# fabiocarrara/neural-ode-features

Measured on AMD Instinct MI355X. Metric: images/sec (fwd+adjoint) CIFAR-10 ODE-ResNet bs=128 at 1/2/4/8 GPU, higher is better.
Workload: dtype f32

## Files before the change

neural-ode-features_amd/csrc/kernels_pointwise.hip:

```cpp
#include "node_internal.h"
#include "wino4.h"
#include "step_control.h"
#include <cstring>
#include "../../include/node_hip.h"

namespace node {


__device__ inline float wave_sum(float v) {
#pragma unroll
  for (int off = 32; off > 0; off >>= 1) v += __shfl_xor(v, off, 64);
  return v;
}
__device__ inline float wave_max(float v) {
#pragma unroll
  for (int off = 32; off > 0; off >>= 1) v = fmaxf(v, __shfl_xor(v, off, 64));
  return v;
}

__device__ inline float block_sum_256(float v, float* red ) {
  v = wave_sum(v);
  __syncthreads();
  if ((threadIdx.x & 63) == 0) red[threadIdx.x >> 6] = v;
  __syncthreads();
// ... 298 lines not shown
struct ErrSegs { ErrSeg seg[3]; float* partial[3]; };
__device__ void error_norm_body(const ErrSeg& seg, const Ctrl* ctrl, float rtol, float atol, float* partial);
__global__ __launch_bounds__(256) void k_error_norm(ErrSegs a, const Ctrl* ctrl, float rtol, float atol) {
  if (ctrl->done) return;
  error_norm_body(a.seg[blockIdx.y], ctrl, rtol, atol, a.partial[blockIdx.y]);
}
__device__ void error_norm_body(const ErrSeg& seg, const Ctrl* ctrl, float rtol, float atol, float* partial) {
  __shared__ float red[4];
  const float dtf = (float)ctrl->dt;
  float ce[7], cb[7];
#pragma unroll
  for (int j = 0; j < 7; ++j) { ce[j] = dtf * c_CERR[j]; cb[j] = dtf * c_CSOL[j]; }
  float acc = 0.f;
  const size_t n4 = seg.n >> 2;
  const size_t stride = (size_t)gridDim.x * 256;
  for (size_t v = (size_t)blockIdx.x * 256 + threadIdx.x; v < n4; v += stride) {
    const size_t off = v * 4;
    float4 kv[7];
#pragma unroll
    for (int j = 0; j < 7; ++j) kv[j] = (j == 1) ? make_float4(0, 0, 0, 0) : ld4(seg.k[j] + off);
    const float4 y0 = ld4(seg.y0 + off);
    float4 y1;
    if (seg.compute_y1) {
      float4 s;
      s.x = cb[0] * kv[0].x; s.y = cb[0] * kv[0].y; s.z = cb[0] * kv[0].z; s.w = cb[0] * kv[0].w;
#pragma unroll
      for (int j = 2; j < 6; ++j) { s.x += cb[j] * kv[j].x; s.y += cb[j] * kv[j].y; s.z += cb[j] * kv[j].z; s.w += cb[j] * kv[j].w; }
      y1 = make_float4(y0.x + s.x, y0.y + s.y, y0.z + s.z, y0.w + s.w);
      st4(seg.y1 + off, y1);
    } else {
// ... 384 lines not shown
  if (!fin) {
    for (int sg = 0; sg < a.nseg; ++sg) {
      const size_t n4 = a.n[sg] >> 2;
      float4* y = reinterpret_cast<float4*>(a.y[sg]);
      const float4* y1 = reinterpret_cast<const float4*>(a.y1[sg]);
      float4* k0 = reinterpret_cast<float4*>(a.k0[sg]);
      const float4* k6 = reinterpret_cast<const float4*>(a.k6[sg]);
      for (size_t i = start; i < n4; i += stride) { y[i] = y1[i]; k0[i] = k6[i]; }
      for (size_t i = (n4 << 2) + start; i < a.n[sg]; i += stride) { a.y[sg][i] = a.y1[sg][i]; a.k0[sg][i] = a.k6[sg][i]; }
    }
    return;
  }
  const float dt = (float)c->dt_used;
  const float t0f = (float)c->t_prev, t1f = (float)c->t;
  const float x = ((float)a.targets[0] - t0f) / (t1f - t0f);
  for (int sg = 0; sg < a.nseg; ++sg)
    for (size_t i = start; i < a.n[sg]; i += stride) {
      float kk[7];
#pragma unroll
      for (int q = 0; q < 7; ++q) kk[q] = (q == 1) ? 0.f : a.k[sg][q][i];
      a.y[sg][i] = interp_one(a.y[sg][i], a.y1[sg][i], kk, dt, x);
    }
}
void launch_commit(const CommitArgs& a, hipStream_t s) {
  size_t nmax = 0;
  for (int i = 0; i < a.nseg; ++i) nmax = a.n[i] > nmax ? a.n[i] : nmax;
  size_t blocks = (nmax / 4 + 255) / 256;
  if (blocks > 2048) blocks = 2048;
  if (blocks < 1) blocks = 1;
  hipLaunchKernelGGL(k_commit, dim3((unsigned)blocks), dim3(256), 0, s, a);
}

__global__ void k_set_target(double* targets, double t_end) { targets[0] = t_end; }
void launch_set_target(double* targets, double t_end, hipStream_t s) {
  hipLaunchKernelGGL(k_set_target, dim3(1), dim3(1), 0, s, targets, t_end);
}
__global__ void k_export_record(const Ctrl* c, node_step_record* r, float* miss_flag, int expect) {
// ... 206 lines not shown
  if (cl == 0) {
    __hip_atomic_store(counter, 0u, __ATOMIC_RELAXED, __HIP_MEMORY_SCOPE_AGENT);
    if (a.write_scalar) a.ctrl->ts_k[a.kidx] = a.osign * tot;
    if (a.vjp_t_out) *a.vjp_t_out = a.osign * tot;
  }
}

void launch_theta_finalize(const Dims& d, const ThetaFinalizeArgs& a, hipStream_t s) {
  size_t wblocks = (9 * (size_t)d.C * d.C / 4 + 255) / 256;
  if (a.dU != nullptr) wblocks = ((size_t)d.C * d.C / 4 + 255) / 256;
  if (wblocks > 1024) wblocks = 1024;
  const size_t nsmall = (9 * (size_t)d.C + 63) / 64;
  hipLaunchKernelGGL(k_theta_finalize, dim3((unsigned)(5 * nsmall + 2 * wblocks)), dim3(256), 0, s, a, d);
}

__global__ __launch_bounds__(256) void k_lincomb(Comb c, const Ctrl* ctrl, float* out, size_t n) {
  const float scale = comb_scale(c, ctrl);
  float cf[7];
#pragma unroll
  for (int j = 0; j < 7; ++j) cf[j] = scale * c.coef[j];
  const size_t stride = (size_t)gridDim.x * 256;
  for (size_t i = (size_t)blockIdx.x * 256 + threadIdx.x; i < n; i += stride) {
    float s = 0.f;
    for (int j = 0; j < c.nk; ++j) s += cf[j] * c.k[j][i];
    out[i] = c.y[i] + s;
  }
}
void launch_lincomb(const Comb& c, const Ctrl* ctrl, float* out, size_t n, hipStream_t s) {
  size_t blocks = (n + 255) / 256;
  if (blocks > 2048) blocks = 2048;
// ... 5 lines not shown
```

neural-ode-features_amd/csrc/node_api.hip:

```cpp
#include "node_internal.h"
#include "wino4.h"
#include "../../include/node_hip.h"

#include <cmath>
#include <cstdarg>
#include <cstdio>
#include <cstring>
#include <cstdlib>
#include <atomic>
#include <mutex>
#include <utility>
#include <vector>

using namespace node;

static thread_local char g_err[512] = "";
static int fail(int code, const char* fmt, ...) {
  va_list ap;
  va_start(ap, fmt);
  vsnprintf(g_err, sizeof(g_err), fmt, ap);
  va_end(ap);
  return code;
}
namespace node {
// ... 202 lines not shown
  unsigned* tcount;
  void* thand;
  float *W4V, *W4M;
  float* w4u[4];
  unsigned short* w4ub[4];
  float* tmapS[2];
  W4Scales* w4sc;
  float* W4Va0b;
  float *W4Va[2], *W4Z[2], *W4dU;
  float *act1b, *xh1b, *r1b;
  float *A, *A1, *KA[7];
  float *TH, *TH1, *KT[7];
  float *xh1, *xh2, *xh3, *r1, *r2, *r3;
  float *dz1, *dz2, *G;
  float *wpart[2], *spart[2], *gpart[3], *sred, *wtime[2];
  float* dots;
  double* targets;
  double* forced;
  double* dtlog;
  size_t bytes;
};
constexpr int STEP_LIST_CAP = 4096;

struct Bump {
  char* base;
  size_t off;
  explicit Bump(void* b) : base((char*)b), off(0) {}
  template <typename T>
  T* take(size_t count) {
    off = (off + 255) & ~(size_t)255;
    T* p = (T*)(base + off);
    off += count * sizeof(T);
    return p;
  }
};

Plan make_plan(const Dims& d, int adjoint, int n_t, void* base) {
  Plan p;
  memset(&p, 0, sizeof(p));
  Bump b(base);
  p.ctrl = b.take<Ctrl>(1);
  p.arrive = b.take<unsigned>(4);
  p.targets = b.take<double>((size_t)(n_t > 0 ? n_t : 1));
  p.forced = b.take<double>(STEP_LIST_CAP);
  p.dtlog = b.take<double>(STEP_LIST_CAP);
  for (int i = 0; i < 3; ++i) p.partial[i] = b.take<float>(ERR_BLOCKS * 2);
  const size_t wsz = conv_packed_elems(d);
  for (int i = 0; i < 2; ++i) p.wf[i] = b.take<float>(wsz);
  for (int i = 0; i < 2; ++i) p.tmap[i] = b.take<float>((size_t)d.HW * d.C);
  p.Y = b.take<float>(d.numel);
// ... 46 lines not shown
    p.r3 = b.take<float>((size_t)d.N * d.G);
    p.dz1 = b.take<float>(d.numel + d.C);
    p.dz2 = b.take<float>(d.numel + d.C);
    p.G = b.take<float>(d.numel);
    for (int i = 0; i < 2; ++i) {
      p.wpart[i] = b.take<float>((size_t)d.nsplit * 9 * d.C * d.C);
      p.spart[i] = b.take<float>(prow * 9 * d.C);
    }
    p.sred = b.take<float>((size_t)2 * 9 * d.C + 2 * ((9 * (size_t)d.C + 63) / 64) + 4);
    for (int i = 0; i < 2; ++i) p.wtime[i] = b.take<float>((size_t)9 * d.C);
    const size_t grows = prow > (size_t)d.mtiles ? prow : (size_t)d.mtiles;
    p.gpart[0] = b.take<float>(grows * 2 * d.C);
    p.gpart[1] = b.take<float>(grows * 2 * d.C);
    p.gpart[2] = b.take<float>(prow * 2 * d.C);
    p.dots = b.take<float>((size_t)(n_t > 0 ? n_t : 1));
  }
  p.bytes = ((b.off + 255) & ~(size_t)255);
  return p;
}

struct HostStage {
  Ctrl* ctrl = nullptr;
  double* lists = nullptr;
  size_t cap = 0;
};
thread_local HostStage g_stage;

int get_stage(size_t doubles, HostStage** out) {
  if (!g_stage.ctrl) HIP_TRY(hipHostMalloc((void**)&g_stage.ctrl, sizeof(Ctrl), hipHostMallocDefault));
  if (g_stage.cap < doubles) {
// ... 92 lines not shown
    if (resident) {
      hipStreamCaptureStatus cs = hipStreamCaptureStatusNone;
      if (hipStreamIsCapturing(st, &cs) != hipSuccess) { (void)hipGetLastError(); cs = hipStreamCaptureStatusNone; }
      if (cs != hipStreamCaptureStatusNone) resident = false;
    }
    if (resident && g_resident_cooldown.load(std::memory_order_relaxed) > 0) {
      g_resident_cooldown.fetch_sub(1, std::memory_order_relaxed);
      resident = false;
    }
  }
  bool w4_b16 = false;
  bool w4_f16 = false;
  bool w4_f16_aug = false;
  SideStream* side = nullptr;
  bool side_pending = false;
  float* va0_of(int set) const { return (set && p.W4Va0b != nullptr) ? p.W4Va0b : p.W4Va[0]; }
  bool g_ready = false;
  bool f16_now() const { return w4_f16 && (!aug || g_ready); }
  bool v_ready = false;
  int cur = 0;
  float* act1_of(int i) const { return i ? p.act1b : p.act1; }
  float* xh1_of(int i) const { return i ? p.xh1b : p.xh1; }
  float* r1_of(int i) const { return i ? p.r1b : p.r1; }
  void to_state(const float* nchw, float* dst) {
    if (w4) launch_w4s_from_nchw(nchw, dst, d.N, d.C, d.w4q, st);
    else launch_nchw_to_nhwc(d, nchw, dst, st);
  }
  void from_state(const float* src, float* nchw) {
    if (w4) launch_w4s_to_nchw(src, nchw, d.N, d.C, d.w4q, st);
    else launch_nhwc_to_nchw(d, src, nchw, st);
// ... 60 lines not shown
    if (tiny_mode() && !w4) {
      launch_tiny_pack(d, prm.conv1_w, p.wtiny[0], st);
      launch_tiny_pack(d, prm.conv2_w, p.wtiny[1], st);
      launch_fill(reinterpret_cast<float*>(p.tcount), 0.f, (size_t)d.N * d.G, st);
    }
    if (w4) {
      w4_b16 = w4_uses_bf16(d.N8, d.C);
      w4_f16 = w4_b16 && w4_f16_fits(d.N8, d.C) && (!aug || (w4_f16_aug && w4_wgrad_on() && w4_wgrad_f16_fits(d.N8, d.C)));
      g_ready = false;
      side = nullptr; side_pending = false;
      if (w4_f16 && aug) {
        const char* e = getenv("NODE_TUNE_W4_WGRAD_SIDE");
        if ((e ? atoi(e) : 0) != 0 && !get_side(&side)) side = nullptr;
      }
      if (w4_f16) { zr[nz] = reinterpret_cast<float*>(p.w4sc); zn[nz++] = sizeof(W4Scales) / sizeof(float); }
    }
    launch_time_prep(d, prm.conv1_w, prm.conv2_w, p.tmap[0], p.tmap[1], aug ? p.wtime[0] : nullptr, aug ? p.wtime[1] : nullptr, zr, zn,
                     nz, st);
    if (w4) {
      W4PackJobs jobs;
      memset(&jobs, 0, sizeof(jobs));
      const float* ws_[4] = {prm.conv1_w, prm.conv2_w, prm.conv1_w, prm.conv2_w};
      if (w4_f16) {
        W4ScaleJobs sj;
        memset(&sj, 0, sizeof(sj));
        sj.w[0] = prm.conv1_w; sj.w[1] = prm.conv2_w; sj.wn = (size_t)d.C * (d.C + 1) * 9;
        sj.gb[0] = prm.norm1_w; sj.gb[1] = prm.norm1_b; sj.gb[2] = prm.norm2_w; sj.gb[3] = prm.norm2_b;
        sj.C = d.C; sj.gn_m = d.cpg * d.HW; sj.sc = p.w4sc;
        launch_w4_scales(sj, st);
      }
// ... 107 lines not shown
    launch_w4s_pass(head, tail, a, st);
  }
  int eval_w4(const Comb& cy, float* y_out, const EvalTime& et, float* kY_out, bool train, const Comb* ca, float* a_out,
              float* kA_out, float* kT_out, int kidx, float csign, float* vjp_t_out, bool need_theta, const NextComb* next) {
    const bool do_aug = ca != nullptr;
    if (next != nullptr)
      for (int j = 0; j + 1 < next->cy.nk; ++j)
        if (next->cy.k[j] == kY_out || (do_aug && next->cy.k[j] == kA_out)) next = nullptr;
    if (!v_ready) {
      W4sArgs a = w4_args();
      w4_tail_combine(a, cy, y_out, train, cur, 0);
      w4_pass(0, 1, a);
    }
    v_ready = false;
    const bool wg4 = do_aug && w4_wgrad_on();
    w4_gemm(0, wg4 ? va0_of(cur) : nullptr);
    {
      W4sArgs a = w4_args();
      a.h.M = p.W4M; a.h.bias = prm.conv1_b; a.h.tmapS = p.tmapS[0]; a.h.et = et; a.h.gamma = prm.norm2_w; a.h.beta = prm.norm2_b;
      a.h.osign = 1.f; a.h.relu = 1;
      if (train) { a.h.out_nhwc = wg4 ? nullptr : p.act2; a.h.xhat_s = p.xh2; a.h.rstd = p.r2; }
      a.V = wg4 ? p.W4Va[1] : p.W4V;
      if (f16_now()) a.v_exp = &p.w4sc->e[W4_E_V2];
      w4_pass(1, 0, a);
    }
    w4_gemm(1, wg4 ? p.W4Va[1] : nullptr);
    W4sArgs a3 = w4_args();
    a3.h.M = p.W4M; a3.h.bias = prm.conv2_b; a3.h.tmapS = p.tmapS[1]; a3.h.et = et; a3.h.gamma = prm.norm3_w; a3.h.beta = prm.norm3_b;
    a3.h.osign = et.tsign; a3.h.relu = 0; a3.h.out_s = kY_out;
    if (!do_aug) {
      if (next != nullptr) {
        const int self = next->cy.nk > 0 && next->cy.k[next->cy.nk - 1] == kY_out;
        w4_tail_combine(a3, next->cy, next->y_out, false, cur, self);
        w4_pass(1, 1, a3);
        v_ready = true;
      } else {
        w4_pass(1, 0, a3);
      }
      if (count_nfe) nfe += 1;
      return check_launch("odefunc forward (F(4x4,3x3))");
    }
    a3.t.comb = *ca; a3.t.csign = csign; a3.t.y_out = a_out; a3.t.gpart = p.gpart[2]; a3.t.spart = p.spart[1];
    if (wg4) a3.t.z_out = need_theta ? p.W4Z[1] : nullptr;
    else a3.t.act_nhwc = p.dz2;
    a3.V = p.W4V;
    if (w4_f16) a3.gstat = p.w4sc;
    if (f16_now()) { a3.v_exp = &p.w4sc->e[W4_E_G]; a3.z_exp = &p.w4sc->e[W4_E_G]; }
    w4_pass(1, 2, a3);
    if (count_nfe) nfe += 1;
    w4_gemm(3);
    {
      W4sArgs a = w4_args();
      a.h.M = p.W4M; a.h.gamma = prm.norm2_w; a.h.beta = prm.norm2_b; a.h.xhat_s = p.xh2; a.h.rstd = p.r2; a.h.osign = 1.f;
      a.h.gpart = p.gpart[1]; a.h.spart = p.spart[0];
      if (wg4) a.h.z_out = need_theta ? p.W4Z[0] : nullptr;
      else a.h.out_nhwc = p.dz1;
      a.V = p.W4V;
      if (w4_f16) a.gstat = p.w4sc;
      if (f16_now()) { a.v_exp = &p.w4sc->e[W4_E_G]; a.z_exp = &p.w4sc->e[W4_E_G]; }
      w4_pass(2, 0, a);
    }
    if (need_theta && wg4 && f16_now()) {
      hipStream_t ws = st;
      if (side != nullptr) {
        (void)hipEventRecord(side->fork, st);
        (void)hipStreamWaitEvent(side->s, side->fork, 0);
        ws = side->s;
      }
      {
        ProfScope ps(1, 2.0 * conv_flops(), ws);
        launch_w4_wgrad_f16(reinterpret_cast<const unsigned*>(va0_of(cur)), reinterpret_cast<const unsigned*>(p.W4Z[0]), reinterpret_cast<const unsigned*>(p.W4Va[1]),
                            reinterpret_cast<const unsigned*>(p.W4Z[1]), p.W4dU, p.ctrl, d.N8, d.C, &p.w4sc->e[W4_E_V1], &p.w4sc->e[W4_E_V2], &p.w4sc->e[W4_E_G], ws);
      }
      if (side != nullptr) { (void)hipEventRecord(side->join, side->s); side_pending = true; }
    } else if (need_theta && wg4) {
      W4WgradArgs wa;
      memset(&wa, 0, sizeof(wa));
      wa.V1 = va0_of(cur); wa.Z1 = p.W4Z[0]; wa.V2 = p.W4Va[1]; wa.Z2 = p.W4Z[1]; wa.dU = p.W4dU; wa.ctrl = p.ctrl; wa.N = d.N8; wa.C = d.C;
      ProfScope ps(1, 2.0 * conv_flops(), st);
      launch_w4_wgrad(wa, st);
    } else if (need_theta) {
      WgradArgs w1;
      memset(&w1, 0, sizeof(w1));
      w1.act = act1_of(cur); w1.dz = p.dz1; w1.wpart = p.wpart[0]; w1.ctrl = p.ctrl;
      if (d.wgrad_pair) { w1.act2 = p.act2; w1.dz2 = p.dz2; w1.wpart2 = p.wpart[1]; }
      { ProfScope ps(1, (d.wgrad_pair ? 2.0 : 1.0) * conv_flops(), st); launch_wgrad(d, w1, st); }
      if (!d.wgrad_pair) {
        WgradArgs w2 = w1;
        w2.act = p.act2; w2.dz = p.dz2; w2.wpart = p.wpart[1];
        { ProfScope ps(1, conv_flops(), st); launch_wgrad(d, w2, st); }
      }
    }
    w4_gemm(2);
    {
      W4sArgs a = w4_args();
      a.h.M = p.W4M; a.h.gamma = prm.norm1_w; a.h.beta = prm.norm1_b; a.h.xhat_s = xh1_of(cur); a.h.rstd = r1_of(cur);
      a.h.osign = et.tsign; a.h.out_s = kA_out; a.h.gpart = p.gpart[0];
      if (next != nullptr) {
        w4_tail_combine(a, next->cy, next->y_out, true, cur ^ 1, 0);
        w4_pass(2, 1, a);
        cur ^= 1;
        v_ready = true;
      } else {
        w4_pass(2, 0, a);
      }
    }
    if (!need_theta) return check_launch("augmented dynamics (F(4x4,3x3))");
    if (side_pending) { (void)hipStreamWaitEvent(st, side->join, 0); side_pending = false; }
    ThetaFinalizeArgs tf;
    memset(&tf, 0, sizeof(tf));
    tf.dU = wg4 ? p.W4dU : nullptr;
    tf.wpart[0] = p.wpart[0]; tf.wpart[1] = p.wpart[1];
    tf.spart[0] = p.spart[0]; tf.spart[1] = p.spart[1];
    tf.gpart[0] = p.gpart[0]; tf.gpart[1] = p.gpart[1]; tf.gpart[2] = p.gpart[2];
    tf.gpart_rows[0] = tf.gpart_rows[1] = tf.gpart_rows[2] = tf.spart_rows = d.N * d.w4q;
    tf.wtime[0] = p.wtime[0]; tf.wtime[1] = p.wtime[1]; tf.sred = p.sred;
    tf.et = et; tf.osign = et.tsign; tf.theta_out = kT_out;
    tf.ctrl = p.ctrl; tf.kidx = kidx; tf.write_scalar = kidx >= 0 ? 1 : 0; tf.vjp_t_out = vjp_t_out;
    launch_theta_finalize(d, tf, st);
    return check_launch("augmented dynamics (F(4x4,3x3))");
  }

  int eval_fwd(const Comb& cy, float* y_out, const EvalTime& et, float* k_out, bool train, const NextComb* next = nullptr) {
// ... 171 lines not shown
    return check_launch("initial step");
  }

  struct StepIO {
    int n_targets = 0;
    int n_forced = 0;
    int log_cap = 0;
    float* y_out = nullptr;
  };

  int enqueue_step(const StepIO& io) {
    static int skip_k2 = -1;
    if (skip_k2 < 0) { const char* e = getenv("NODE_TUNE_SKIP_K2_THETA"); skip_k2 = e ? atoi(e) : 1; }
    const bool was_counting = count_nfe;
    count_nfe = false;
    for (int s = 0; s < 6; ++s) {
      const int rc = eval_sys(s + 1, DP_BETA[s], s + 1, SC_DT, et_stage(DP_ALPHA[s]), s == 5, !(skip_k2 && s == 0),
                              s < 5 ? DP_BETA[s + 1] : nullptr, s + 2, s + 1 == 5);
      if (rc != NODE_OK) { count_nfe = was_counting; return rc; }
    }
    count_nfe = was_counting;
    const int nseg = aug ? 3 : 1;
    ErrSeg es[3];
    es[0].y0 = p.Y; es[0].y1 = p.Y1; es[0].n = d.numel; es[0].compute_y1 = 0;
    for (int j = 0; j < 7; ++j) es[0].k[j] = p.KY[j];
    if (aug) {
      es[1] = es[0];
      es[1].y0 = p.A; es[1].y1 = p.A1;
      for (int j = 0; j < 7; ++j) es[1].k[j] = p.KA[j];
      es[2].y0 = p.TH; es[2].y1 = p.TH1; es[2].n = d.P; es[2].compute_y1 = 1;
      for (int j = 0; j < 7; ++j) es[2].k[j] = p.KT[j];
    }
    StepCtlArgs sc;
    memset(&sc, 0, sizeof(sc));
    sc.ctrl = p.ctrl;
    sc.partial[0] = p.partial[0]; sc.partial[1] = p.partial[1]; sc.partial[2] = p.partial[2];
    sc.numel[0] = (double)d.numel; sc.numel[1] = (double)d.numel; sc.numel[2] = (double)d.P;
    sc.nseg = nseg; sc.has_scalar = aug ? 1 : 0; sc.rtol = rtol; sc.atol = atol;
    sc.targets = p.targets; sc.n_targets = io.n_targets;
    sc.forced = io.n_forced > 0 ? p.forced : nullptr; sc.n_forced = io.n_forced;
    sc.dt_log = io.log_cap > 0 ? p.dtlog : nullptr; sc.dt_log_cap = io.log_cap;
    sc.interp_scalar = aug ? 1 : 0;
    sc.w4sc = (aug && w4_f16) ? p.w4sc : nullptr;
    if (nr_fn == nullptr && fold_ctl()) {
      launch_error_norm_ctl(es, p.partial, nseg, sc, p.arrive, st);
    } else {
// ... 6 lines not shown
      ea.ctrl = p.ctrl; ea.targets = p.targets; ea.y0 = p.Y; ea.y1 = p.Y1;
      for (int j = 0; j < 7; ++j) ea.k[j] = p.KY[j];
      ea.y_out = io.y_out;
      if (w4) launch_w4s_emit_outputs(d, ea, st);
      else launch_emit_outputs(d, ea, st);
    }
    CommitArgs cm;
    memset(&cm, 0, sizeof(cm));
    cm.ctrl = p.ctrl; cm.targets = p.targets; cm.nseg = nseg; cm.interp_final = aug ? 1 : 0;
    cm.y[0] = p.Y; cm.y1[0] = p.Y1; cm.k0[0] = p.KY[0]; cm.k6[0] = p.KY[6]; cm.n[0] = d.numel;
    for (int j = 0; j < 7; ++j) cm.k[0][j] = p.KY[j];
    if (aug) {
      cm.y[1] = p.A; cm.y1[1] = p.A1; cm.k0[1] = p.KA[0]; cm.k6[1] = p.KA[6]; cm.n[1] = d.numel;
      cm.y[2] = p.TH; cm.y1[2] = p.TH1; cm.k0[2] = p.KT[0]; cm.k6[2] = p.KT[6]; cm.n[2] = d.P;
      for (int j = 0; j < 7; ++j) { cm.k[1][j] = p.KA[j]; cm.k[2][j] = p.KT[j]; }
    }
    launch_commit(cm, st);
    return check_launch("dopri5 step");
  }

  int run_steps(const StepIO& io, long long max_steps, int guess, int* status) {
    long long enq = 0;
    long long batch = guess > 0 ? guess : 1;
    for (;;) {
      if (batch > max_steps - enq) batch = max_steps - enq;
      for (long long i = 0; i < batch; ++i) TRY(enqueue_step(io));
      enq += batch;
      TRY(readback());
      if (hctrl->status != 0) { *status = hctrl->status; return NODE_OK; }
      if (hctrl->done) return NODE_OK;
// ... 840 lines not shown
  hipStream_t st = (hipStream_t)stream;
  const int nseg = f->nseg, aug = f->has_scalar ? 1 : 0;
  if (method == NODE_METHOD_RK4) {
    const double cf[4] = {1.0 / 8, 3.0 / 8, 3.0 / 8, 1.0 / 8};
    for (int i = 0; i < nseg; ++i) {
      float* ks[7];
      for (int j = 0; j < 7; ++j) ks[j] = f->seg[i].k[j];
      launch_lincomb(Solver::make_comb(f->seg[i].y, ks, cf, 4, SC_DT), p.ctrl, f->seg[i].y1, f->seg[i].n, st);
      HIP_TRY(hipMemcpyAsync(f->seg[i].y, f->seg[i].y1, f->seg[i].n * sizeof(float), hipMemcpyDeviceToDevice, st));
    }
    if (aug) launch_set_scalar_state(p.ctrl, 0.f, 1, st);
    return flat_launch_ok("node_flat_finish_step(rk4)");
  }
  if (method != NODE_METHOD_DOPRI5) return fail(NODE_ERR_ARG, "unknown method %d", method);
  ErrSeg es[3];
  for (int i = 0; i < nseg; ++i) {
    es[i].y0 = f->seg[i].y; es[i].y1 = f->seg[i].y1; es[i].n = f->seg[i].n; es[i].compute_y1 = 0;
    for (int j = 0; j < 7; ++j) es[i].k[j] = f->seg[i].k[j];
  }
  launch_error_norm(es, p.partial, nseg, p.ctrl, f->rtol, f->atol, st);
  StepCtlArgs sc;
  memset(&sc, 0, sizeof(sc));
  sc.ctrl = p.ctrl;
  for (int i = 0; i < nseg; ++i) { sc.partial[i] = p.partial[i]; sc.numel[i] = (double)f->seg[i].n; }
  sc.nseg = nseg; sc.has_scalar = aug; sc.rtol = f->rtol; sc.atol = f->atol;
  sc.targets = p.targets; sc.n_targets = f->n_targets; sc.interp_scalar = aug;
  launch_step_controller(sc, st);
  if (y_out != nullptr) {
    EmitArgs ea;
    ea.ctrl = p.ctrl; ea.targets = p.targets; ea.y0 = f->seg[0].y; ea.y1 = f->seg[0].y1;
// ... 139 lines not shown
```

neural-ode-features_amd/csrc/node_internal.h:

```cpp
#pragma once
#include <hip/hip_runtime.h>
#include <stdint.h>
#include <stddef.h>

namespace node {

constexpr int KCH = 32;
constexpr int BN = 64;
constexpr int WG_THREADS = 256;

struct Dims {
  int N, C, H, W, HW, G, cpg;
  float eps;
  int Wp, Hp, SLOTS;
  int MARGIN;
  int BNE;
  int ntile;
  int nchunk;
  int BM;
  int S;
  int wino;
  int wgrad_wino;
  int wut;
  int tiny;
// ... 75 lines not shown
};
__device__ inline float comb_scale(const Comb& c, const Ctrl* ctrl) {
  return c.scale_mode == SC_ABS ? 1.0f : (c.scale_mode == SC_DT ? (float)ctrl->dt : ctrl->h0);
}

__device__ constexpr float DP_CMID_F[7] = {
    (float)(6025192743.0 / 30085553152.0 / 2.0), 0.f, (float)(51252292925.0 / 65400821598.0 / 2.0),
    (float)(-2691868925.0 / 45128329728.0 / 2.0), (float)(187940372067.0 / 1594534317056.0 / 2.0),
    (float)(-1776094331.0 / 19743644256.0 / 2.0), (float)(11237099.0 / 235043384.0 / 2.0)};
__device__ inline float interp_one(float y0, float y1, const float* k, float dt, float x) {
  float s = (dt * DP_CMID_F[0]) * k[0];
#pragma unroll
  for (int j = 2; j < 7; ++j) s += (dt * DP_CMID_F[j]) * k[j];
  const float ymid = y0 + s;
  const float f0 = k[0], f1 = k[6];
  const float ca = (-2.f * dt) * f0 + (2.f * dt) * f1 + -8.f * y0 + -8.f * y1 + 16.f * ymid;
  const float cb = (5.f * dt) * f0 + (-3.f * dt) * f1 + 18.f * y0 + 14.f * y1 + -32.f * ymid;
  const float cc = (-4.f * dt) * f0 + dt * f1 + -11.f * y0 + -5.f * y1 + 16.f * ymid;
  const float cd = dt * f0;
  const float x2 = x * x, x3 = x2 * x, x4 = x3 * x;
  return ca * x4 + cb * x3 + cc * x2 + cd * x + y0;
}

constexpr int MAX_DEVICES = 64;
inline void allow_full_lds(const void* fn, bool (&done)[MAX_DEVICES]) {
  int dev = 0;
  (void)hipGetDevice(&dev);
  const bool tracked = dev >= 0 && dev < MAX_DEVICES;
  if (tracked && done[dev]) return;
  if (hipFuncSetAttribute(fn, hipFuncAttributeMaxDynamicSharedMemorySize, 160 * 1024) != hipSuccess)
// ... 81 lines not shown
  const float* gamma;
  float* dz_out;
  float* gpart;
  float* spart;
  const float* mask_act;
  float osign;
};
void launch_gn_bwd(const Dims& d, const GnBwdArgs& a, hipStream_t s);

struct ErrSeg {
  const float* y0;
  float* y1;
  const float* k[7];
  size_t n;
  int compute_y1;
};
constexpr int ERR_BLOCKS = 512;
void launch_error_norm(const ErrSeg* segs, float* const* partial , int nseg, const Ctrl* ctrl, float rtol, float atol, hipStream_t s);
struct StepCtlArgs;
void launch_error_norm_ctl(const ErrSeg* segs, float* const* partial, int nseg, const StepCtlArgs& ctl, unsigned* arrive, hipStream_t s);

struct StepCtlArgs {
  Ctrl* ctrl;
  const float* partial[3];
  double numel[3];
  int nseg;
  int has_scalar;
  float rtol, atol;
  const double* targets;
  int n_targets;
// ... 24 lines not shown
  const float* y0; const float* y1; const float* k[7];
  float* y_out;
};
void launch_emit_outputs(const Dims& d, const EmitArgs& a, hipStream_t s);
void launch_emit_flat(const EmitArgs& a, size_t n, hipStream_t s);
void launch_flat_time(const EvalTime& et, float* out, hipStream_t s);
void launch_flat_scalar(Ctrl* ctrl, int which, const float* src, float scale, int accumulate, hipStream_t s);
struct CommitArgs {
  const Ctrl* ctrl;
  const double* targets;
  int nseg;
  float* y[3]; const float* y1[3]; float* k0[3]; const float* k6[3];
  const float* k[3][7];
  size_t n[3];
  int interp_final;
};
void launch_commit(const CommitArgs& a, hipStream_t s);
void launch_set_interval(Ctrl* ctrl, double t, double dt, hipStream_t s);
void launch_set_target(double* targets, double t_end, hipStream_t s);
}
struct node_step_record;
namespace node {
void launch_export_record(const Ctrl* ctrl, node_step_record* rec, float* miss_flag, int expect_steps, hipStream_t s);

struct InitSeg { const float* y0; const float* f0; const float* f1; size_t n; };
void launch_init_norms(const InitSeg* segs, float* const* partial , int nseg, float rtol, float atol, int phase, hipStream_t s);
struct InitCtlArgs;
void launch_init_norms_ctl(const InitSeg* segs, float* const* partial, int nseg, const InitCtlArgs& ctl, unsigned* arrive, hipStream_t s);
struct InitCtlArgs {
  Ctrl* ctrl;
// ... 73 lines not shown
  const float* spart[2];
  const float* gpart[3];
  int gpart_rows[3];
  int spart_rows;
  const float* wtime[2];
  float* sred;
  EvalTime et;
  float osign;
  float* theta_out;
  Ctrl* ctrl;
  int kidx;
  int write_scalar;
  float* vjp_t_out;
};
void launch_theta_finalize(const Dims& d, const ThetaFinalizeArgs& a, hipStream_t s);

struct TinyConvArgs {
  const float* act;
  const unsigned short* wq;
  const float* bias; const float* tmap;
  EvalTime et;
  const float* gamma; const float* beta;
  float* out;
  float* part; unsigned* counter;
  const Ctrl* ctrl;
  int relu; float osign;
  int nx_on, nx_self;
  Comb nx; float* nx_y_out; const float* nx_gamma; const float* nx_beta; float* nx_act;
};
struct TinyResidentArgs {
// ... 54 lines not shown
```

Before: 28120.

## Batch theta finalize across Dopri5 stages into one fused step kernel

In the adjoint step, the per-stage theta-gradient finalize (Winograd dU back-transform plus GN and bias reductions) is deferred. Each stage writes into its own slot buffers, and one kernel then reduces all five stages at once and emits theta1, the error, the midpoint combination and k6 directly. The error-norm and commit kernels gain fast paths that read these precomputed err and mid arrays instead of reloading all seven k vectors for theta. This removes five per-stage finalize launches and repeated passes over the parameter-sized buffers, at the cost of extra workspace per stage and a gfx950-only fence-free hand-off.

```diff
diff --git a/neural-ode-features_amd/csrc/kernels_pointwise.hip b/neural-ode-features_amd/csrc/kernels_pointwise.hip
--- a/neural-ode-features_amd/csrc/kernels_pointwise.hip
+++ b/neural-ode-features_amd/csrc/kernels_pointwise.hip
@@ -336,6 +336,28 @@
   float acc = 0.f;
   const size_t n4 = seg.n >> 2;
   const size_t stride = (size_t)gridDim.x * 256;
+  if (seg.err != nullptr) {
+    for (size_t v = (size_t)blockIdx.x * 256 + threadIdx.x; v < n4; v += stride) {
+      const size_t off = v * 4;
+      const float4 y0 = ld4(seg.y0 + off), y1 = ld4(seg.y1 + off), e = ld4(seg.err + off);
+      float r;
+      r = e.x / (atol + rtol * fmaxf(fabsf(y0.x), fabsf(y1.x))); acc += r * r;
+      r = e.y / (atol + rtol * fmaxf(fabsf(y0.y), fabsf(y1.y))); acc += r * r;
+      r = e.z / (atol + rtol * fmaxf(fabsf(y0.z), fabsf(y1.z))); acc += r * r;
+      r = e.w / (atol + rtol * fmaxf(fabsf(y0.w), fabsf(y1.w))); acc += r * r;
+      acc += 0.f * (((y0.x + y0.y) + (y0.z + y0.w)) + ((y1.x + y1.y) + (y1.z + y1.w)));
+    }
+    if (blockIdx.x == 0)
+      for (size_t i = (n4 << 2) + threadIdx.x; i < seg.n; i += 256) {
+        const float y0 = seg.y0[i], y1 = seg.y1[i];
+        const float r = seg.err[i] / (atol + rtol * fmaxf(fabsf(y0), fabsf(y1)));
+        acc += r * r;
+        acc += 0.f * (y0 + y1);
+      }
+    const float tot = block_sum_256(acc, red);
+    if (threadIdx.x == 0) __hip_atomic_store(&partial[blockIdx.x], tot, __ATOMIC_RELAXED, __HIP_MEMORY_SCOPE_AGENT);
+    return;
+  }
   for (size_t v = (size_t)blockIdx.x * 256 + threadIdx.x; v < n4; v += stride) {
     const size_t off = v * 4;
     float4 kv[7];
@@ -750,13 +772,19 @@
   const float dt = (float)c->dt_used;
   const float t0f = (float)c->t_prev, t1f = (float)c->t;
   const float x = ((float)a.targets[0] - t0f) / (t1f - t0f);
-  for (int sg = 0; sg < a.nseg; ++sg)
+  for (int sg = 0; sg < a.nseg; ++sg) {
+    if (a.mid[sg] != nullptr) {
+      for (size_t i = start; i < a.n[sg]; i += stride)
+        a.y[sg][i] = interp_mid(a.y[sg][i], a.y1[sg][i], a.k[sg][0][i], a.k[sg][6][i], a.mid[sg][i], dt, x);
+      continue;
+    }
     for (size_t i = start; i < a.n[sg]; i += stride) {
       float kk[7];
 #pragma unroll
       for (int q = 0; q < 7; ++q) kk[q] = (q == 1) ? 0.f : a.k[sg][q][i];
       a.y[sg][i] = interp_one(a.y[sg][i], a.y1[sg][i], kk, dt, x);
     }
+  }
 }
 void launch_commit(const CommitArgs& a, hipStream_t s) {
   size_t nmax = 0;
@@ -993,6 +1021,174 @@
   hipLaunchKernelGGL(k_theta_finalize, dim3((unsigned)(5 * nsmall + 2 * wblocks)), dim3(256), 0, s, a, d);
 }
 
+__device__ const float c_W4_GF[6][3] = {{(float)W4_G[0][0], (float)W4_G[0][1], (float)W4_G[0][2]}, {(float)W4_G[1][0], (float)W4_G[1][1], (float)W4_G[1][2]},
+                                        {(float)W4_G[2][0], (float)W4_G[2][1], (float)W4_G[2][2]}, {(float)W4_G[3][0], (float)W4_G[3][1], (float)W4_G[3][2]},
+                                        {(float)W4_G[4][0], (float)W4_G[4][1], (float)W4_G[4][2]}, {(float)W4_G[5][0], (float)W4_G[5][1], (float)W4_G[5][2]}};
+__device__ inline void theta_step_emit(const ThetaStepArgs& a, size_t idx, const float* k, float dtf) {
+  const float k0 = a.k0[idx];
+  float sb = c_CSOL[0] * k0, se = c_CERR[0] * k0, sm = DP_CMID_F[0] * k0;
+#pragma unroll
+  for (int s = 0; s < TH_STAGES; ++s) { sb += c_CSOL[2 + s] * k[s]; se += c_CERR[2 + s] * k[s]; sm += DP_CMID_F[2 + s] * k[s]; }
+  a.th1[idx] = a.th[idx] + dtf * sb;
+  a.err[idx] = dtf * se;
+  a.mid[idx] = dtf * sm;
+  a.k6[idx] = k[TH_STAGES - 1];
+}
+__global__ __launch_bounds__(256) void k_theta_finalize_step(ThetaStepArgs a, Dims d) {
+  if (a.ctrl->done) return;
+  __shared__ float red[TH_STAGES][256];
+  __shared__ int s_last;
+  const ThetaLayout L = theta_layout(d.C);
+  const int C = d.C;
+  const float dtf = (float)a.ctrl->dt;
+  const int nsm = (9 * C + 63) / 64;
+  const int bx_all = blockIdx.x;
+  const int wb = ((int)gridDim.x - 5 * nsm) / 2;
+  if (bx_all >= 5 * nsm) {
+    const int layer = (bx_all - 5 * nsm) / wb, bx = (bx_all - 5 * nsm) - layer * wb;
+    const size_t CC = (size_t)C * C, cc2 = CC / 2;
+    const size_t stride = (size_t)wb * 256;
+    const size_t base = L.wc[layer];
+    for (size_t i = (size_t)bx * 256 + threadIdx.x; i < cc2; i += stride) {
+      float2 ob[9], oe[9], om[9], o6[9];
+#pragma unroll
+      for (int q = 0; q < 9; ++q) ob[q] = oe[q] = om[q] = o6[q] = make_float2(0.f, 0.f);
+#pragma unroll 1
+      for (int xi = 0; xi < 6; ++xi) {
+        float2 ub[6], ue[6], um[6], u6[6];
+#pragma unroll
+        for (int nu = 0; nu < 6; ++nu) ub[nu] = ue[nu] = um[nu] = u6[nu] = make_float2(0.f, 0.f);
+#pragma unroll
+        for (int s = 0; s < TH_STAGES; ++s)
+#pragma unroll
+          for (int nu = 0; nu < 6; ++nu) {
+            const float2 u = reinterpret_cast<const float2*>(a.dU[s] + (size_t)layer * W4_COMPS * CC)[(size_t)(xi * 6 + nu) * cc2 + i];
+            ub[nu].x += c_CSOL[2 + s] * u.x; ub[nu].y += c_CSOL[2 + s] * u.y;
+            ue[nu].x += c_CERR[2 + s] * u.x; ue[nu].y += c_CERR[2 + s] * u.y;
+            um[nu].x += DP_CMID_F[2 + s] * u.x; um[nu].y += DP_CMID_F[2 + s] * u.y;
+            if (s == TH_STAGES - 1) u6[nu] = u;
+          }
+        const float gh[3] = {c_W4_GF[xi][0], c_W4_GF[xi][1], c_W4_GF[xi][2]};
+#pragma unroll
+        for (int kw = 0; kw < 3; ++kw) {
+          float2 tb = make_float2(0.f, 0.f), te = tb, tm = tb, t6 = tb;
+#pragma unroll
+          for (int nu = 0; nu < 6; ++nu) {
+            const float gq = (float)W4_G[nu][kw];
+            if (gq != 0.f) {
+              tb.x += gq * ub[nu].x; tb.y += gq * ub[nu].y; te.x += gq * ue[nu].x; te.y += gq * ue[nu].y;
+              tm.x += gq * um[nu].x; tm.y += gq * um[nu].y; t6.x += gq * u6[nu].x; t6.y += gq * u6[nu].y;
+            }
+          }
+#pragma unroll
+          for (int kh = 0; kh < 3; ++kh) {
+            const int q = kh * 3 + kw;
+            ob[q].x += gh[kh] * tb.x; ob[q].y += gh[kh] * tb.y; oe[q].x += gh[kh] * te.x; oe[q].y += gh[kh] * te.y;
+            om[q].x += gh[kh] * tm.x; om[q].y += gh[kh] * tm.y; o6[q].x += gh[kh] * t6.x; o6[q].y += gh[kh] * t6.y;
+          }
+        }
+      }
+#pragma unroll
+      for (int q = 0; q < 9; ++q) {
+        const size_t idx = base + (size_t)q * CC + 2 * i;
+        const float2 k0 = *reinterpret_cast<const float2*>(a.k0 + idx), th = *reinterpret_cast<const float2*>(a.th + idx);
+        float2 v;
+        v.x = th.x + dtf * (c_CSOL[0] * k0.x + a.tsign * ob[q].x); v.y = th.y + dtf * (c_CSOL[0] * k0.y + a.tsign * ob[q].y);
+        *reinterpret_cast<float2*>(a.th1 + idx) = v;
+        v.x = dtf * (c_CERR[0] * k0.x + a.tsign * oe[q].x); v.y = dtf * (c_CERR[0] * k0.y + a.tsign * oe[q].y);
+        *reinterpret_cast<float2*>(a.err + idx) = v;
+        v.x = dtf * (DP_CMID_F[0] * k0.x + a.tsign * om[q].x); v.y = dtf * (DP_CMID_F[0] * k0.y + a.tsign * om[q].y);
+        *reinterpret_cast<float2*>(a.mid + idx) = v;
+        v.x = a.tsign * o6[q].x; v.y = a.tsign * o6[q].y;
+        *reinterpret_cast<float2*>(a.k6 + idx) = v;
+      }
+    }
+    return;
+  }
+  const int job = bx_all / nsm, bxs = bx_all - job * nsm;
+  const bool gn = job < 3;
+  const int layer = gn ? job : job - 3;
+  const int ncol = gn ? 2 * C : 9 * C;
+  if (bxs * 64 >= ncol) return;
+  const int rows = a.rows;
+  const int cl = threadIdx.x & 63, rg = threadIdx.x >> 6;
+  const int col = bxs * 64 + cl;
+#pragma unroll
+  for (int s = 0; s < TH_STAGES; ++s) {
+    const float* src = gn ? a.gpart[s][layer] : a.spart[s][layer];
+    float v = 0.f;
+    if (col < ncol) {
+      int r = rg;
+      for (; r + 12 < rows; r += 16) {
+        const float v0 = src[(size_t)r * ncol + col], v1 = src[(size_t)(r + 4) * ncol + col];
+        const float v2 = src[(size_t)(r + 8) * ncol + col], v3 = src[(size_t)(r + 12) * ncol + col];
+        v += (v0 + v1) + (v2 + v3);
+      }
+      for (; r < rows; r += 4) v += src[(size_t)r * ncol + col];
+    }
+    red[s][threadIdx.x] = v;
+  }
+  __syncthreads();
+  if (rg != 0) return;
+  const bool on = col < ncol;
+  float v[TH_STAGES], k[TH_STAGES];
+#pragma unroll
+  for (int s = 0; s < TH_STAGES; ++s) v[s] = (red[s][cl] + red[s][64 + cl]) + (red[s][128 + cl] + red[s][192 + cl]);
+  if (gn) {
+    if (on) {
+      const int which = col >= C ? 1 : 0;
+#pragma unroll
+      for (int s = 0; s < TH_STAGES; ++s) k[s] = a.tsign * v[s];
+      theta_step_emit(a, (which ? L.b[layer] : L.g[layer]) + (col - which * C), k, dtf);
+    }
+    return;
+  }
+  if (on) {
+    const float tf = (float)a.ctrl->t;
+#pragma unroll
+    for (int s = 0; s < TH_STAGES; ++s) k[s] = a.tsign * (v[s] * (a.tsign * (tf + a.alpha[s] * dtf)));
+    theta_step_emit(a, L.wt[layer] + col, k, dtf);
+    if (col >= 4 * C && col < 5 * C) {
+#pragma unroll
+      for (int s = 0; s < TH_STAGES; ++s) k[s] = a.tsign * v[s];
+      theta_step_emit(a, L.cb[layer] + (col - 4 * C), k, dtf);
+    }
+  }
+  const int nb = nsm;
+  float* dotpart = a.dotpart;
+  unsigned* counter = reinterpret_cast<unsigned*>(dotpart + TH_STAGES * 2 * nb);
+  const float wt = on ? a.wtime[layer][col] : 0.f;
+  float part[TH_STAGES];
+#pragma unroll
+  for (int s = 0; s < TH_STAGES; ++s) part[s] = wave_sum(on ? v[s] * wt : 0.f);
+#if defined(__HIP_DEVICE_COMPILE__) && !defined(__gfx950__)
+#error "k_theta_finalize_step's fence-free hand-off is only valid on gfx950: use release/acquire on the counter elsewhere"
+#endif
+  if (cl == 0) {
+#pragma unroll
+    for (int s = 0; s < TH_STAGES; ++s)
+      __hip_atomic_store(dotpart + (s * 2 + layer) * nb + bxs, part[s], __ATOMIC_RELAXED, __HIP_MEMORY_SCOPE_AGENT);
+    asm volatile("s_waitcnt vmcnt(0)" ::: "memory");
+    s_last = __hip_atomic_fetch_add(counter, 1u, __ATOMIC_RELAXED, __HIP_MEMORY_SCOPE_AGENT) == (unsigned)(2 * nb - 1);
+  }
+  __builtin_amdgcn_wave_barrier();
+  if (!s_last) return;
+  for (int s = 0; s < TH_STAGES; ++s) {
+    float tot = 0.f;
+    for (int i = cl; i < 2 * nb; i += 64) tot += __hip_atomic_load(dotpart + s * 2 * nb + i, __ATOMIC_RELAXED, __HIP_MEMORY_SCOPE_AGENT);
+    tot = wave_sum(tot);
+    if (cl == 0) a.ctrl->ts_k[2 + s] = a.tsign * tot;
+  }
+  if (cl == 0) __hip_atomic_store(counter, 0u, __ATOMIC_RELAXED, __HIP_MEMORY_SCOPE_AGENT);
+}
+
+void launch_theta_finalize_step(const Dims& d, const ThetaStepArgs& a, hipStream_t s) {
+  size_t wblocks = ((size_t)d.C * d.C / 2 + 255) / 256;
+  if (wblocks > 1024) wblocks = 1024;
+  const size_t nsmall = (9 * (size_t)d.C + 63) / 64;
+  hipLaunchKernelGGL(k_theta_finalize_step, dim3((unsigned)(5 * nsmall + 2 * wblocks)), dim3(256), 0, s, a, d);
+}
+
 __global__ __launch_bounds__(256) void k_lincomb(Comb c, const Ctrl* ctrl, float* out, size_t n) {
   const float scale = comb_scale(c, ctrl);
   float cf[7];
diff --git a/neural-ode-features_amd/csrc/node_api.hip b/neural-ode-features_amd/csrc/node_api.hip
--- a/neural-ode-features_amd/csrc/node_api.hip
+++ b/neural-ode-features_amd/csrc/node_api.hip
@@ -240,6 +240,7 @@
   float *xh1, *xh2, *xh3, *r1, *r2, *r3;
   float *dz1, *dz2, *G;
   float *wpart[2], *spart[2], *gpart[3], *sred, *wtime[2];
+  float *dUs[TH_STAGES], *sparts[TH_STAGES][2], *gparts[TH_STAGES][3], *THerr, *THmid, *thdot;
   float* dots;
   double* targets;
   double* forced;
@@ -260,6 +261,8 @@
     return p;
   }
 };
+
+static bool theta_batch_fits(const Dims& d) { return d.wino4 && d.C % 128 == 0 && d.C < 512; }
 
 Plan make_plan(const Dims& d, int adjoint, int n_t, void* base) {
   Plan p;
@@ -336,6 +339,18 @@
     p.gpart[1] = b.take<float>(grows * 2 * d.C);
     p.gpart[2] = b.take<float>(prow * 2 * d.C);
     p.dots = b.take<float>((size_t)(n_t > 0 ? n_t : 1));
+    if (theta_batch_fits(d) && p.W4dU != nullptr) {
+      for (int s = 0; s < TH_STAGES; ++s) {
+        p.dUs[s] = b.take<float>(w4_du_elems(d.C));
+        for (int i = 0; i < 2; ++i) p.sparts[s][i] = b.take<float>(prow * 9 * d.C);
+        p.gparts[s][0] = b.take<float>(grows * 2 * d.C);
+        p.gparts[s][1] = b.take<float>(grows * 2 * d.C);
+        p.gparts[s][2] = b.take<float>(prow * 2 * d.C);
+      }
+      p.THerr = b.take<float>(d.P);
+      p.THmid = b.take<float>(d.P);
+      p.thdot = b.take<float>((size_t)TH_STAGES * 2 * ((9 * (size_t)d.C + 63) / 64) + 4);
+    }
   }
   p.bytes = ((b.off + 255) & ~(size_t)255);
   return p;
@@ -458,6 +473,8 @@
   bool w4_f16_aug = false;
   SideStream* side = nullptr;
   bool side_pending = false;
+  bool theta_batch = false;
+  int th_slot = -1;
   float* va0_of(int set) const { return (set && p.W4Va0b != nullptr) ? p.W4Va0b : p.W4Va[0]; }
   bool g_ready = false;
   bool f16_now() const { return w4_f16 && (!aug || g_ready); }
@@ -548,6 +565,12 @@
         if ((e ? atoi(e) : 0) != 0 && !get_side(&side)) side = nullptr;
       }
       if (w4_f16) { zr[nz] = reinterpret_cast<float*>(p.w4sc); zn[nz++] = sizeof(W4Scales) / sizeof(float); }
+      theta_batch = false; th_slot = -1;
+      if (w4_f16 && aug && p.dUs[0] != nullptr) {
+        const char* e = getenv("NODE_TUNE_W4_THETA_BATCH");
+        theta_batch = (e ? atoi(e) : 1) != 0;
+      }
+      if (theta_batch) { zr[nz] = p.thdot + (size_t)TH_STAGES * 2 * ((9 * (size_t)d.C + 63) / 64); zn[nz++] = 1; }
     }
     launch_time_prep(d, prm.conv1_w, prm.conv2_w, p.tmap[0], p.tmap[1], aug ? p.wtime[0] : nullptr, aug ? p.wtime[1] : nullptr, zr, zn,
                      nz, st);
@@ -685,6 +708,10 @@
     }
     v_ready = false;
     const bool wg4 = do_aug && w4_wgrad_on();
+    const bool slot = wg4 && need_theta && th_slot >= 0;
+    float* const dU_out = slot ? p.dUs[th_slot] : p.W4dU;
+    float* const* gp = slot ? p.gparts[th_slot] : p.gpart;
+    float* const* sp = slot ? p.sparts[th_slot] : p.spart;
     w4_gemm(0, wg4 ? va0_of(cur) : nullptr);
     {
       W4sArgs a = w4_args();
@@ -711,7 +738,7 @@
       if (count_nfe) nfe += 1;
       return check_launch("odefunc forward (F(4x4,3x3))");
     }
-    a3.t.comb = *ca; a3.t.csign = csign; a3.t.y_out = a_out; a3.t.gpart = p.gpart[2]; a3.t.spart = p.spart[1];
+    a3.t.comb = *ca; a3.t.csign = csign; a3.t.y_out = a_out; a3.t.gpart = gp[2]; a3.t.spart = sp[1];
     if (wg4) a3.t.z_out = need_theta ? p.W4Z[1] : nullptr;
     else a3.t.act_nhwc = p.dz2;
     a3.V = p.W4V;
@@ -723,7 +750,7 @@
     {
       W4sArgs a = w4_args();
       a.h.M = p.W4M; a.h.gamma = prm.norm2_w; a.h.beta = prm.norm2_b; a.h.xhat_s = p.xh2; a.h.rstd = p.r2; a.h.osign = 1.f;
-      a.h.gpart = p.gpart[1]; a.h.spart = p.spart[0];
+      a.h.gpart = gp[1]; a.h.spart = sp[0];
       if (wg4) a.h.z_out = need_theta ? p.W4Z[0] : nullptr;
       else a.h.out_nhwc = p.dz1;
       a.V = p.W4V;
@@ -741,13 +768,13 @@
       {
         ProfScope ps(1, 2.0 * conv_flops(), ws);
         launch_w4_wgrad_f16(reinterpret_cast<const unsigned*>(va0_of(cur)), reinterpret_cast<const unsigned*>(p.W4Z[0]), reinterpret_cast<const unsigned*>(p.W4Va[1]),
-                            reinterpret_cast<const unsigned*>(p.W4Z[1]), p.W4dU, p.ctrl, d.N8, d.C, &p.w4sc->e[W4_E_V1], &p.w4sc->e[W4_E_V2], &p.w4sc->e[W4_E_G], ws);
+                            reinterpret_cast<const unsigned*>(p.W4Z[1]), dU_out, p.ctrl, d.N8, d.C, &p.w4sc->e[W4_E_V1], &p.w4sc->e[W4_E_V2], &p.w4sc->e[W4_E_G], ws);
       }
       if (side != nullptr) { (void)hipEventRecord(side->join, side->s); side_pending = true; }
     } else if (need_theta && wg4) {
       W4WgradArgs wa;
       memset(&wa, 0, sizeof(wa));
-      wa.V1 = va0_of(cur); wa.Z1 = p.W4Z[0]; wa.V2 = p.W4Va[1]; wa.Z2 = p.W4Z[1]; wa.dU = p.W4dU; wa.ctrl = p.ctrl; wa.N = d.N8; wa.C = d.C;
+      wa.V1 = va0_of(cur); wa.Z1 = p.W4Z[0]; wa.V2 = p.W4Va[1]; wa.Z2 = p.W4Z[1]; wa.dU = dU_out; wa.ctrl = p.ctrl; wa.N = d.N8; wa.C = d.C;
       ProfScope ps(1, 2.0 * conv_flops(), st);
       launch_w4_wgrad(wa, st);
     } else if (need_theta) {
@@ -766,7 +793,7 @@
     {
       W4sArgs a = w4_args();
       a.h.M = p.W4M; a.h.gamma = prm.norm1_w; a.h.beta = prm.norm1_b; a.h.xhat_s = xh1_of(cur); a.h.rstd = r1_of(cur);
-      a.h.osign = et.tsign; a.h.out_s = kA_out; a.h.gpart = p.gpart[0];
+      a.h.osign = et.tsign; a.h.out_s = kA_out; a.h.gpart = gp[0];
       if (next != nullptr) {
         w4_tail_combine(a, next->cy, next->y_out, true, cur ^ 1, 0);
         w4_pass(2, 1, a);
@@ -778,6 +805,7 @@
     }
     if (!need_theta) return check_launch("augmented dynamics (F(4x4,3x3))");
     if (side_pending) { (void)hipStreamWaitEvent(st, side->join, 0); side_pending = false; }
+    if (slot) return check_launch("augmented dynamics (F(4x4,3x3))");
     ThetaFinalizeArgs tf;
     memset(&tf, 0, sizeof(tf));
     tf.dU = wg4 ? p.W4dU : nullptr;
@@ -979,14 +1007,32 @@
     if (skip_k2 < 0) { const char* e = getenv("NODE_TUNE_SKIP_K2_THETA"); skip_k2 = e ? atoi(e) : 1; }
     const bool was_counting = count_nfe;
     count_nfe = false;
+    const bool tb = aug && theta_batch && skip_k2;
     for (int s = 0; s < 6; ++s) {
+      th_slot = (tb && s >= 1) ? s - 1 : -1;
       const int rc = eval_sys(s + 1, DP_BETA[s], s + 1, SC_DT, et_stage(DP_ALPHA[s]), s == 5, !(skip_k2 && s == 0),
                               s < 5 ? DP_BETA[s + 1] : nullptr, s + 2, s + 1 == 5);
-      if (rc != NODE_OK) { count_nfe = was_counting; return rc; }
-    }
+      if (rc != NODE_OK) { count_nfe = was_counting; th_slot = -1; return rc; }
+    }
+    th_slot = -1;
     count_nfe = was_counting;
+    if (tb) {
+      ThetaStepArgs ts;
+      memset(&ts, 0, sizeof(ts));
+      for (int s = 0; s < TH_STAGES; ++s) {
+        ts.dU[s] = p.dUs[s];
+        ts.spart[s][0] = p.sparts[s][0]; ts.spart[s][1] = p.sparts[s][1];
+        ts.gpart[s][0] = p.gparts[s][0]; ts.gpart[s][1] = p.gparts[s][1]; ts.gpart[s][2] = p.gparts[s][2];
+        ts.alpha[s] = (float)DP_ALPHA[s + 1];
+      }
+      ts.rows = d.N * d.w4q;
+      ts.wtime[0] = p.wtime[0]; ts.wtime[1] = p.wtime[1]; ts.dotpart = p.thdot; ts.tsign = tsign;
+      ts.th = p.TH; ts.k0 = p.KT[0]; ts.th1 = p.TH1; ts.err = p.THerr; ts.mid = p.THmid; ts.k6 = p.KT[6]; ts.ctrl = p.ctrl;
+      launch_theta_finalize_step(d, ts, st);
+    }
     const int nseg = aug ? 3 : 1;
     ErrSeg es[3];
+    memset(es, 0, sizeof(es));
     es[0].y0 = p.Y; es[0].y1 = p.Y1; es[0].n = d.numel; es[0].compute_y1 = 0;
     for (int j = 0; j < 7; ++j) es[0].k[j] = p.KY[j];
     if (aug) {
@@ -995,6 +1041,7 @@
       for (int j = 0; j < 7; ++j) es[1].k[j] = p.KA[j];
       es[2].y0 = p.TH; es[2].y1 = p.TH1; es[2].n = d.P; es[2].compute_y1 = 1;
       for (int j = 0; j < 7; ++j) es[2].k[j] = p.KT[j];
+      if (tb) { es[2].compute_y1 = 0; es[2].err = p.THerr; }
     }
     StepCtlArgs sc;
     memset(&sc, 0, sizeof(sc));
@@ -1031,6 +1078,7 @@
       cm.y[1] = p.A; cm.y1[1] = p.A1; cm.k0[1] = p.KA[0]; cm.k6[1] = p.KA[6]; cm.n[1] = d.numel;
       cm.y[2] = p.TH; cm.y1[2] = p.TH1; cm.k0[2] = p.KT[0]; cm.k6[2] = p.KT[6]; cm.n[2] = d.P;
       for (int j = 0; j < 7; ++j) { cm.k[1][j] = p.KA[j]; cm.k[2][j] = p.KT[j]; }
+      if (tb) cm.mid[2] = p.THmid;
     }
     launch_commit(cm, st);
     return check_launch("dopri5 step");
@@ -1901,6 +1949,7 @@
   }
   if (method != NODE_METHOD_DOPRI5) return fail(NODE_ERR_ARG, "unknown method %d", method);
   ErrSeg es[3];
+  memset(es, 0, sizeof(es));
   for (int i = 0; i < nseg; ++i) {
     es[i].y0 = f->seg[i].y; es[i].y1 = f->seg[i].y1; es[i].n = f->seg[i].n; es[i].compute_y1 = 0;
     for (int j = 0; j < 7; ++j) es[i].k[j] = f->seg[i].k[j];
diff --git a/neural-ode-features_amd/csrc/node_internal.h b/neural-ode-features_amd/csrc/node_internal.h
--- a/neural-ode-features_amd/csrc/node_internal.h
+++ b/neural-ode-features_amd/csrc/node_internal.h
@@ -113,6 +113,15 @@
   for (int j = 2; j < 7; ++j) s += (dt * DP_CMID_F[j]) * k[j];
   const float ymid = y0 + s;
   const float f0 = k[0], f1 = k[6];
+  const float ca = (-2.f * dt) * f0 + (2.f * dt) * f1 + -8.f * y0 + -8.f * y1 + 16.f * ymid;
+  const float cb = (5.f * dt) * f0 + (-3.f * dt) * f1 + 18.f * y0 + 14.f * y1 + -32.f * ymid;
+  const float cc = (-4.f * dt) * f0 + dt * f1 + -11.f * y0 + -5.f * y1 + 16.f * ymid;
+  const float cd = dt * f0;
+  const float x2 = x * x, x3 = x2 * x, x4 = x3 * x;
+  return ca * x4 + cb * x3 + cc * x2 + cd * x + y0;
+}
+__device__ inline float interp_mid(float y0, float y1, float f0, float f1, float mid, float dt, float x) {
+  const float ymid = y0 + mid;
   const float ca = (-2.f * dt) * f0 + (2.f * dt) * f1 + -8.f * y0 + -8.f * y1 + 16.f * ymid;
   const float cb = (5.f * dt) * f0 + (-3.f * dt) * f1 + 18.f * y0 + 14.f * y1 + -32.f * ymid;
   const float cc = (-4.f * dt) * f0 + dt * f1 + -11.f * y0 + -5.f * y1 + 16.f * ymid;
@@ -224,6 +233,7 @@
   const float* k[7];
   size_t n;
   int compute_y1;
+  const float* err;
 };
 constexpr int ERR_BLOCKS = 512;
 void launch_error_norm(const ErrSeg* segs, float* const* partial , int nseg, const Ctrl* ctrl, float rtol, float atol, hipStream_t s);
@@ -278,6 +288,7 @@
   const float* k[3][7];
   size_t n[3];
   int interp_final;
+  const float* mid[3];
 };
 void launch_commit(const CommitArgs& a, hipStream_t s);
 void launch_set_interval(Ctrl* ctrl, double t, double dt, hipStream_t s);
@@ -381,6 +392,25 @@
   float* vjp_t_out;
 };
 void launch_theta_finalize(const Dims& d, const ThetaFinalizeArgs& a, hipStream_t s);
+constexpr int TH_STAGES = 5;
+struct ThetaStepArgs {
+  const float* dU[TH_STAGES];
+  const float* spart[TH_STAGES][2];
+  const float* gpart[TH_STAGES][3];
+  int rows;
+  const float* wtime[2];
+  float* dotpart;
+  float alpha[TH_STAGES];
+  float tsign;
+  const float* th;
+  const float* k0;
+  float* th1;
+  float* err;
+  float* mid;
+  float* k6;
+  Ctrl* ctrl;
+};
+void launch_theta_finalize_step(const Dims& d, const ThetaStepArgs& a, hipStream_t s);
 
 struct TinyConvArgs {
   const float* act;
```

Result: no change. 28150 (median of 4 runs) (+0.1%).
